# ORNL/HydraGNN

Measured on NVIDIA H100. Metric: atoms_per_sec_training_step, higher is better.
Workload: dtype tf32

## Files before the change

### hydragnn_b200/ops.py

```python
import torch
from torch.autograd.function import once_differentiable

from . import _lib

ACT_CODES = {None: 0, "none": 0, "relu": 1, "silu": 2, "tanh": 3, "sigmoid": 4, "lrelu": 5, "elu": 6, "selu": 7}
POOL_CODES = {"add": 0, "sum": 0, "mean": 1, "max": 2}


def _stream():
    return torch.cuda.current_stream().cuda_stream


def _p(t):
    return None if t is None else t.data_ptr()


def _chk(t, dtype=torch.float32):
    if t is None:
        return None
    if not t.is_cuda:
        raise RuntimeError("hydragnn_b200 ops need CUDA tensors (no CPU fallback on the hot path)")
    if t.dtype != dtype:
        raise RuntimeError("expected %s, got %s" % (dtype, t.dtype))
    return t if t.is_contiguous() else t.contiguous()
# ... 578 lines not shown
                                                leaves=ctx.leaves2)
            gx, gw1, gb1 = linear_bwd_dispatch(dz1, x2, w1, ctx.needs_input_grad[0], ctx.needs_input_grad[1],
                                               has_b1 and ctx.needs_input_grad[2], leaves=ctx.leaves1)
        return (gx.reshape(shp) if gx is not None else None), gw1, gb1, None, None, gw2, gb2, None, None


class Mlp2ScalarFn(torch.autograd.Function):

    @staticmethod
    def forward(ctx, x, w1, b1, act1, p1, w2, b2):
        n, out = x.shape[0], w2.shape[0]
        pad = x.new_zeros(4 - out)
        pk = torch.cat([w1.reshape(1), b1.reshape(1), w2.reshape(out), pad, b2.reshape(out), pad]).contiguous()
        x1 = _chk(x.reshape(n).contiguous())
        y = torch.empty(n, out, dtype=x.dtype, device=x.device)
        _lib.call("hgb_mlp2_scalar_fwd", _p(x1), _p(pk), n, out, ACT_CODES[act1], float(p1), _p(y), _stream())
        ctx.save_for_backward(x1, pk)
        ctx.cfg = (ACT_CODES[act1], float(p1), out)
        return y

    @staticmethod
    @once_differentiable
    def backward(ctx, gy):
        x1, pk = ctx.saved_tensors
        code, p1, out = ctx.cfg
        n = x1.shape[0]
        gx = torch.empty_like(x1) if ctx.needs_input_grad[0] else None
        gp = torch.empty(10, dtype=x1.dtype, device=x1.device)
        ws = _ws(_lib.query("hgb_mlp2_scalar_workspace_bytes"), x1.device)
        _lib.call("hgb_mlp2_scalar_bwd", _p(_chk(gy.contiguous())), _p(x1), _p(pk), n, out, code, p1, _p(gx), _p(gp), _p(ws), _stream())
        return (gx.reshape(n, 1) if gx is not None else None), gp[0:1].reshape(1, 1), gp[1:2], None, None, gp[2:2 + out].reshape(out, 1), gp[6:6 + out]


def mlp2(x, w1, b1, act1, p1, w2, b2, act2=None, p2=0.0):
    if (act2 is None and b1 is not None and b2 is not None and x.dim() == 2 and x.shape[1] == 1
            and w1.shape == (1, 1) and w2.shape[1] == 1 and w2.shape[0] <= 4):
        return Mlp2ScalarFn.apply(x, w1, b1, act1, p1, w2, b2)
    return Mlp2Fn.apply(x, w1, b1, act1, p1, w2, b2, act2, p2)


class EdgeGeomFn(torch.autograd.Function):

    @staticmethod
    def forward(ctx, pos, shifts, plan, eps):
        pos = _chk(pos)
        e = plan.num_edges
        vec = torch.empty(e, 3, dtype=pos.dtype, device=pos.device)
        ln = torch.empty(e, 1, dtype=pos.dtype, device=pos.device)
        unit = torch.empty(e, 3, dtype=pos.dtype, device=pos.device)
        _lib.call("hgb_edge_geom_fwd", _p(pos), _p(plan.row), _p(plan.col), _p(_chk(shifts)), e, float(eps), _p(vec), _p(ln),
                  _p(unit), _stream())
        ctx.save_for_backward(vec, ln)
        ctx.plan, ctx.eps = plan, float(eps)
        return vec, ln, unit

    @staticmethod
    @once_differentiable
    def backward(ctx, g_vec, g_len, g_unit):
        vec, ln = ctx.saved_tensors
        plan = ctx.plan
        gv = torch.empty_like(vec)
        _lib.call("hgb_edge_geom_bwd", _p(vec), _p(ln), ctx.eps, _p(_chk(g_vec)), _p(_chk(g_len)), _p(_chk(g_unit)),
                  plan.num_edges, _p(gv), _stream())
        g_pos = g_shift = None
        if ctx.needs_input_grad[0]:
            g_pos = raw_segment_sum(gv, plan.by_col.rowptr, plan.by_col.perm, plan.num_nodes) - \
                raw_segment_sum(gv, plan.by_row.rowptr, plan.by_row.perm, plan.num_nodes)
        if ctx.needs_input_grad[1]:
            g_shift = gv
        return g_pos, g_shift, None, None
# ... 60 lines not shown
            key = epack.data_ptr()
            if key not in cache:
                cache.clear()
                cache[key] = painn_edge_records(epack, plan, "col")
            rec_col = cache[key]
        _lib.call("hgb_painn_message_bwd", _p(gs_out), _p(gv_out), _p(phi), _p(v), _p(src.rowptr), _p(src.perm), _p(plan.nbr("col")),
                  _p(epack), _p(rec_col), _p(wf), _p(bf), _p(efilt), n, f, r, _p(gphi), _p(gv), _p(gwf), _p(gbf), _p(g_epack), _p(g_ef),
                  _p(ws), nbytes, _stream())
        return gphi, gs_out, gv, g_epack, gwf, gbf, g_ef, None, None


def painn_edge_records(epack, plan, which):
    csr = plan.by_row if which == "row" else plan.by_col
    rec = torch.empty(plan.num_edges, 16, dtype=epack.dtype, device=epack.device)
    _lib.call("hgb_painn_edge_records", _p(epack.detach()), _p(csr.perm), _p(plan.nbr(which)), plan.num_edges, _p(rec), _stream())
    return rec


def raw_linear(x2, w, b, code=0, param=0.0, want_z=False):
    m, k = x2.shape
    n = w.shape[0]
    y = torch.empty(m, n, dtype=x2.dtype, device=x2.device)
    z = torch.empty_like(y) if want_z else None
    _lib.call("hgb_linear_fwd", _p(x2), _p(w), _p(b), m, n, k, x2.stride(0), w.stride(0), code, float(param), _p(y), _p(z), _stream())
    return y, z


def raw_act_bwd(dy, y, z, code, param=0.0):
    dz = torch.empty_like(dy)
    _lib.call("hgb_act_bwd", _p(dy), _p(y), _p(z), dy.numel(), code, float(param), _p(dz), _stream())
    return dz


class PainnUpdateFn(torch.autograd.Function):

    @staticmethod
    def forward(ctx, s, v, uw, ub, vw, vb, w1, b1, w2, b2, last):
        n, f = s.shape
        s, v = _chk(s), _chk(v)
        w1, b1, w2, b2 = [_chk(t) for t in (w1, b1, w2, b2)]
        v2 = v.reshape(3 * n, f)
        wuv, buv = torch.cat([uw, vw], dim=0).contiguous(), torch.cat([ub, vb], dim=0).contiguous()
        y_uv, _ = linear_fwd_dispatch(v2, wuv, buv)
        uv, vv, ld = y_uv, y_uv[:, f:], 2 * f
        mlp_in = torch.empty(n, 2 * f, dtype=s.dtype, device=s.device)
        _lib.call("hgb_painn_update_pre_fwd", _p(vv), ld, _p(s), n, f, _p(mlp_in), _stream())
        h, z1, deriv = linear_fwd_dispatch_ex(mlp_in, w1, b1, ACT_CODES["silu"], 0.0, want_z=True, z_deriv=True)
        a, _ = linear_fwd_dispatch(h, w2, b2)
        ctx.z1_code = ACT_DERIV if deriv else ACT_CODES["silu"]
        s_out = torch.empty_like(s)
        v_out = None if last else torch.empty_like(v)
        _lib.call("hgb_painn_update_post_fwd", _p(a), _p(uv), _p(vv), ld, _p(s), _p(v), n, f, int(last), _p(s_out), _p(v_out), _stream())
        ctx.save_for_backward(v2, y_uv, mlp_in, z1, h, a, wuv, w1, w2)
        ctx.last = bool(last)
        ctx.tc = _TC["enabled"]
        ctx.leaves = ([uw, ub, vw, vb], [w1, b1], [w2, b2])
        if last:
            return s_out, s_out.new_zeros(0)
        return s_out, v_out

    @staticmethod
    @once_differentiable
    def backward(ctx, gs_out, gv_out):
        v2, y_uv, mlp_in, z1, h, a, wuv, w1, w2 = ctx.saved_tensors
        last = ctx.last
        n, f = gs_out.shape
        ld = 2 * f
        uv, vv = y_uv, y_uv[:, f:]
        gs_out = _chk(gs_out)
        gv_out = None if last else _chk(gv_out.contiguous())
        ga = torch.empty_like(a)
        _lib.call("hgb_painn_update_post_bwd_a", _p(gs_out), _p(gv_out), _p(uv), _p(vv), ld, n, f, int(last), _p(ga), _stream())
        with tensor_cores(ctx.tc):
            gz1, gw2, gb2 = linear_bwd_dispatch(ga, h, w2, dx_gsrc=z1, dx_gact=ctx.z1_code, leaves=ctx.leaves[2])
            g_mlp_in, gw1, gb1 = linear_bwd_dispatch(gz1, mlp_in, w1, leaves=ctx.leaves[1])
        g_uv = torch.empty_like(y_uv)
        gs = torch.empty_like(gs_out)
        _lib.call("hgb_painn_update_bwd", _p(gs_out), _p(gv_out), _p(g_mlp_in), _p(a), _p(uv), _p(vv), ld, _p(mlp_in), n, f,
                  int(last), _p(g_uv), _p(g_uv[:, f:]), _p(gs), None, _stream())
        with tensor_cores(ctx.tc):
            gv, gwuv, gbuv = linear_bwd_dispatch(g_uv, v2, wuv, dx_addend=None if last else gv_out.reshape(3 * n, f), leaves=ctx.leaves[0])
        return gs, gv.reshape(n, 3, f), gwuv[:f], gbuv[:f], gwuv[f:], gbuv[f:], gw1, gb1, gw2, gb2, None


def painn_update_tc_ok(s, v):
    n, f = s.shape
    return (_TC["enabled"] and f == 64 and tuple(v.shape) == (n, 3, f) and s.is_cuda and v.is_cuda
            and s.dtype == torch.float32 and v.dtype == torch.float32 and s.is_contiguous() and v.is_contiguous()
            and s.data_ptr() % 16 == 0 and v.data_ptr() % 16 == 0 and bool(_lib.query("hgb_tc_linear_supported", n, f, 2 * f)))


def _aligned(t):
    t = _chk(t)
    return t if t.data_ptr() % 16 == 0 else t.clone()


class PainnUpdateTcFn(torch.autograd.Function):

    @staticmethod
    def forward(ctx, s, v, uw, ub, vw, vb, w1, b1, w2, b2, last):
        n, f = s.shape
        w1, b1, w2, b2 = [_chk(t) for t in (w1, b1, w2, b2)]
        wuv, buv = torch.cat([uw, vw], dim=0).contiguous(), torch.cat([ub, vb], dim=0).contiguous()
        mlp_in = torch.empty(n, 2 * f, dtype=s.dtype, device=s.device)
        inner = torch.empty_like(s) if last else None
        _lib.call("hgb_painn_update_tc_fwd", _p(v), _p(s), _p(wuv), _p(buv), n, _p(mlp_in), _p(inner), _stream())
        h, z1, deriv = linear_fwd_dispatch_ex(mlp_in, w1, b1, ACT_CODES["silu"], 0.0, want_z=True, z_deriv=True)
        a, _ = linear_fwd_dispatch(h, w2, b2)
        ctx.z1_code = ACT_DERIV if deriv else ACT_CODES["silu"]
        s_out = torch.empty_like(s)
        v_out = None if last else torch.empty_like(v)
        _lib.call("hgb_painn_update_tc_post", _p(v), _p(s), _p(a), _p(inner), _p(wuv), _p(buv), n, int(last), _p(s_out), _p(v_out),
                  _stream())
        ctx.save_for_backward(v, mlp_in, z1, h, a, wuv, buv, w1, w2, inner)
        ctx.last = bool(last)
        ctx.leaves = ([uw, ub, vw, vb], [w1, b1], [w2, b2])
        if last:
            return s_out, s_out.new_zeros(0)
        return s_out, v_out

    @staticmethod
    @once_differentiable
    def backward(ctx, gs_out, gv_out):
        v, mlp_in, z1, h, a, wuv, buv, w1, w2, inner = ctx.saved_tensors
        last = ctx.last
        n, f = mlp_in.shape[0], v.shape[2]
        gs_out = _aligned(gs_out)
        gv_out = None if last else _aligned(gv_out)
        ga = torch.empty_like(a)
        _lib.call("hgb_painn_update_tc_bwd_a", _p(v), _p(gs_out), _p(gv_out), _p(inner), _p(wuv), _p(buv), n, int(last), _p(ga), _stream())
        with tensor_cores(True):
            gz1, gw2, gb2 = linear_bwd_dispatch(ga, h, w2, dx_gsrc=z1, dx_gact=ctx.z1_code, leaves=ctx.leaves[2])
            g_mlp_in, gw1, gb1 = linear_bwd_dispatch(gz1, mlp_in, w1, leaves=ctx.leaves[1])
        g_uv = torch.empty(3 * n, 2 * f, dtype=v.dtype, device=v.device)
        gs, gv = torch.empty_like(gs_out), torch.empty_like(v)
        _lib.call("hgb_painn_update_tc_bwd", _p(v), _p(gs_out), _p(gv_out), _p(g_mlp_in), _p(a), _p(mlp_in), _p(wuv), _p(buv), n, int(last),
                  _p(g_uv), _p(gs), _p(gv), _stream())
        with tensor_cores(True):
            _, gwuv, gbuv = linear_bwd_dispatch(g_uv, v.reshape(3 * n, f), wuv, need_x=False, leaves=ctx.leaves[0])
        return gs, gv, gwuv[:f], gbuv[:f], gwuv[f:], gbuv[f:], gw1, gb1, gw2, gb2, None


class PainnUpdateScalarFn(torch.autograd.Function):

    @staticmethod
    def forward(ctx, s, v, uw, ub, vw, vb, w1, b1, w2, b2, last):
        n = s.shape[0]
        na = 2 if last else 3
        pad = s.new_zeros(3 - na)
        pk = torch.cat([uw.reshape(1), ub.reshape(1), vw.reshape(1), vb.reshape(1), w1.reshape(2), b1.reshape(1), w2.reshape(na), pad,
                        b2.reshape(na), pad, s.new_zeros(3)]).contiguous()
        s2, v2 = _chk(s.reshape(n).contiguous()), _chk(v.reshape(n, 3).contiguous())
        s_out = torch.empty_like(s2)
        v_out = None if last else torch.empty_like(v2)
        _lib.call("hgb_painn_update_scalar_fwd", _p(s2), _p(v2), _p(pk), n, int(last), _p(s_out), _p(v_out), _stream())
        ctx.save_for_backward(s2, v2, pk)
        ctx.last = bool(last)
        if last:
            return s_out.reshape(n, 1), s_out.new_zeros(0)
        return s_out.reshape(n, 1), v_out.reshape(n, 3, 1)

    @staticmethod
    @once_differentiable
    def backward(ctx, gs_out, gv_out):
        s2, v2, pk = ctx.saved_tensors
        n, last = s2.shape[0], ctx.last
# ... 679 lines not shown
```

### include/hgb.h

```cpp
#ifndef HGB_H
#define HGB_H

#include <stdint.h>

#ifdef __cplusplus
extern "C" {
#endif

typedef void* hgb_stream_t;

#define HGB_OK 0
#define HGB_EINVAL (-1)
#define HGB_ECUDA (-2)
#define HGB_ECAPACITY (-3)

#define HGB_ACT_DERIV 100
#define HGB_ACT_NONE 0
#define HGB_ACT_RELU 1
#define HGB_ACT_SILU 2
#define HGB_ACT_TANH 3
#define HGB_ACT_SIGMOID 4
#define HGB_ACT_LRELU 5
#define HGB_ACT_ELU 6
#define HGB_ACT_SELU 7
// ... 58 lines not shown
int hgb_segment_argminmax(const float* m, const int32_t* rowptr, const int32_t* perm, int32_t n, int32_t c,
                          int64_t* argmin, int64_t* argmax, hgb_stream_t stream);
int hgb_pool_fwd(const float* x, const int32_t* graph_ptr, int32_t g, int32_t c, int32_t mode,
                 float* out, int32_t* argmax, hgb_stream_t stream);
int hgb_pool_bwd(const float* gout, const int32_t* graph_ptr, const int32_t* argmax, int32_t n,
                 int32_t g, int32_t c, int32_t mode, float* gx, hgb_stream_t stream);


int hgb_gemm(const float* a, const float* b, float* c, int32_t m, int32_t n, int32_t k,
             int32_t trans_a, int32_t trans_b, int64_t lda, int64_t ldb, int64_t ldc, int32_t beta_one,
             void* workspace, int64_t workspace_bytes, hgb_stream_t stream);
int64_t hgb_gemm_workspace_bytes(int32_t m, int32_t n, int32_t k, int32_t trans_a);
int hgb_linear_fwd(const float* x, const float* w, const float* b, int32_t m, int32_t n, int32_t k,
                   int64_t ldx, int64_t ldw, int32_t act, float act_param, float* y, float* z,
                   hgb_stream_t stream);
int hgb_linear_smallk_supported(int32_t n, int32_t k);
int hgb_linear_smallk_fwd(const float* x, int64_t ldx, const float* w, int64_t ldw, const float* b, int32_t m,
                          int32_t n, int32_t k, int32_t act, float act_param, float* y, float* z,
                          hgb_stream_t stream);
int hgb_linear_smallk_bwd(const float* dy, const float* y, const float* z, const float* x, int64_t ldx,
                          const float* w, int64_t ldw, int32_t m, int32_t n, int32_t k, int32_t act,
                          float act_param, float* dx, float* dw, int64_t lddw, float* db, void* workspace,
                          hgb_stream_t stream);
int64_t hgb_linear_smallk_bwd_workspace_bytes(int32_t m, int32_t n, int32_t k);

int hgb_tc_linear_supported(int32_t m, int32_t n_out, int32_t k_red);
int hgb_tc_linear(const float* a, int64_t lda, const float* w, int64_t ldw, int32_t trans_b, const float* bias,
                  int32_t m, int32_t n_out, int32_t k_red, int32_t act, float act_param, float* y, float* z,
                  const float* addend, const float* gsrc, int32_t gact, int32_t exact, hgb_stream_t stream);
int hgb_tc_wgrad(const float* dz, int64_t lddz, const float* x, int64_t ldx, int32_t m, int32_t n_out,
                 int32_t k_out, float* dw, int64_t lddw, float* db, int32_t accumulate, int32_t exact,
                 void* workspace, int64_t workspace_bytes, hgb_stream_t stream);
int64_t hgb_tc_wgrad_workspace_bytes(int32_t n_out, int32_t k_out);
int hgb_act_bwd(const float* dy, const float* y, const float* z, int64_t count, int32_t act,
                float act_param, float* dz, hgb_stream_t stream);
int hgb_act_deriv(const float* x, int64_t count, int32_t act, float act_param, int32_t order,
                  float* out, hgb_stream_t stream);
int hgb_colsum(const float* x, int32_t m, int32_t n, float* out, void* workspace, hgb_stream_t stream);
int64_t hgb_colsum_workspace_bytes(int32_t m, int32_t n);


int hgb_edge_geom_fwd(const float* pos, const int32_t* row, const int32_t* col, const float* shifts,
                      int64_t e, float eps, float* vec, float* len, float* unit, hgb_stream_t stream);
int hgb_edge_geom_bwd(const float* vec, const float* len, float eps, const float* g_vec_in,
                      const float* g_len, const float* g_unit, int64_t e, float* g_vec,
                      hgb_stream_t stream);
int hgb_painn_edge_embed_fwd(const float* unit, const float* len, int64_t e, int32_t r, float cutoff,
                             float* epack, hgb_stream_t stream);
int hgb_painn_edge_embed_bwd(const float* unit, const float* len, const float* g_epack, int64_t e, int32_t r,
                             float cutoff, float* g_unit, float* g_len, hgb_stream_t stream);


int hgb_painn_message_fwd(const float* phi, const float* s, const float* v, const int32_t* rowptr,
                          const int32_t* perm, const int32_t* nbr, const float* epack, const float* rec,
                          const float* wf, const float* bf, const float* efilt, int32_t n, int32_t f, int32_t r,
                          float* s_out, float* v_out, hgb_stream_t stream);
int hgb_painn_edge_records(const float* epack, const int32_t* perm, const int32_t* nbr, int64_t e, float* rec,
                           hgb_stream_t stream);
int hgb_painn_message_bwd(const float* gs_out, const float* gv_out, const float* phi, const float* v,
                          const int32_t* rowptr_src, const int32_t* perm_src, const int32_t* nbr_agg,
                          const float* epack, const float* rec, const float* wf, const float* bf, const float* efilt, int32_t n,
                          int32_t f, int32_t r, float* gphi, float* gv, float* gwf, float* gbf, float* g_epack,
                          float* g_efilt, void* workspace, int64_t workspace_bytes, hgb_stream_t stream);
int64_t hgb_painn_message_bwd_workspace_bytes(int32_t n, int32_t f, int32_t r);

int hgb_painn_update_pre_fwd(const float* vv, int64_t ld, const float* s, int32_t n, int32_t f, float* mlp_in,
// ... 152 lines not shown
```

### profiles/kbench.py

```python
import os, sys, json
sys.path.insert(0, os.path.dirname(os.path.dirname(os.path.abspath(__file__))))
import torch
import hydragnn_b200 as hb
from hydragnn_b200 import ops
from hydragnn_b200.stacks import Base
from hydragnn_b200.synthetic import ARCH, make_samples

dev = torch.device("cuda")
flush = torch.empty(256 * 1024 * 1024, dtype=torch.uint8, device=dev)


def timeit(fn, iters=10, warm=3):
    ts = []
    for it in range(iters + warm):
        flush.zero_()
        a, b = torch.cuda.Event(enable_timing=True), torch.cuda.Event(enable_timing=True)
        a.record(); fn(); b.record(); torch.cuda.synchronize()
        if it >= warm:
            ts.append(a.elapsed_time(b))
    return sum(ts) / len(ts)


def tc_linear_calls(n):
    silu, tanh, deriv = ops.ACT_CODES["silu"], ops.ACT_CODES["tanh"], ops.ACT_DERIV
# ... 21 lines not shown
        res["tc_linear %s m=%d (ms | GB/s)" % (name, m)] = (round(t, 4), round(nbytes / t / 1e6, 1))
    return res


def painn_update_calls(n, f=64):
    from hydragnn_b200.stacks import PainnUpdate
    units = {("fused", True): (19, 44), ("fused", False): (25, 56), ("unfused", True): (32, 58), ("unfused", False): (40, 72)}
    U = n * f * 4
    res = {}
    overlap = ops.WGRAD_OVERLAP
    ops.WGRAD_OVERLAP = False
    try:
        for last in (True, False):
            upd = PainnUpdate(f, last).to(dev)
            params = [upd.update_U.weight, upd.update_U.bias, upd.update_V.weight, upd.update_V.bias, upd.update_mlp[0].weight,
                      upd.update_mlp[0].bias, upd.update_mlp[2].weight, upd.update_mlp[2].bias]
            s = torch.randn(n, f, device=dev, requires_grad=True)
            v = torch.randn(n, 3, f, device=dev, requires_grad=True)
            for kind, fn in (("fused", ops.PainnUpdateTcFn), ("unfused", ops.PainnUpdateFn)):
                with ops.tensor_cores(True):
                    so, vo = fn.apply(s, v, *params, last)
                    outs = (so,) if last else (so, vo)
                    grads = tuple(torch.randn_like(o) for o in outs)
                    t_f = timeit(lambda: fn.apply(s, v, *params, last))
                    t_b = timeit(lambda: torch.autograd.grad(outs, [s, v] + params, grads, retain_graph=True))
                uf, ub = units[(kind, last)]
                res["painn_update %s last=%s fwd (ms | GB/s | U)" % (kind, last)] = (round(t_f, 4), round(uf * U / t_f / 1e6, 1), uf)
                res["painn_update %s last=%s bwd (ms | GB/s | U)" % (kind, last)] = (round(t_b, 4), round(ub * U / t_b / 1e6, 1), ub)
    finally:
        ops.WGRAD_OVERLAP = overlap
    return res


G = 16384
b = make_samples("qm9_painn", G).to(dev); b._num_graphs = G
if os.environ.get("KBENCH_ONLY") == "tc_linear":
    print(json.dumps(tc_linear_calls(b.pos.shape[0]), indent=1)); sys.exit(0)
if os.environ.get("KBENCH_ONLY") == "painn_update":
    print(json.dumps(painn_update_calls(b.pos.shape[0]), indent=1)); sys.exit(0)
b = hb.get_radius_graph(7.0, 5)(b)
plan = Base.plan_for(b)
n, e, f, r = plan.num_nodes, plan.num_edges, 64, 5
_, ln, unit = ops.EdgeGeomFn.apply(b.pos, None, plan, 1e-9)
epack = ops.PainnEdgeEmbedFn.apply(unit, ln, r, 7.0)
s, v, phi = torch.randn(n, f, device=dev), torch.randn(n, 3, f, device=dev), torch.randn(n, 3 * f, device=dev)
wf, bf = torch.randn(3 * f, r, device=dev), torch.randn(3 * f, device=dev)
out = {}
rec = ops.painn_edge_records(epack, plan, "row")
out["painn_message_fwd F=64 (ms)"] = timeit(lambda: ops.PainnMessageFn.apply(phi, s, v, epack, wf, bf, None, plan, rec))
out["painn_edge_records (ms)"] = timeit(lambda: ops.painn_edge_records(epack, plan, "row"))
sr, vr, pr = s.clone().requires_grad_(True), v.clone().requires_grad_(True), phi.clone().requires_grad_(True)
so, vo = ops.PainnMessageFn.apply(pr, sr, vr, epack, wf.requires_grad_(True), bf.requires_grad_(True), None, plan, rec)
gs, gv = torch.randn_like(so), torch.randn_like(vo)
out["painn_message_bwd F=64 (ms)"] = timeit(lambda: torch.autograd.grad((so, vo), (pr, sr, vr, wf, bf), (gs, gv), retain_graph=True))
so2, vo2 = ops.PainnMessageFn.apply(pr, sr, vr, epack, wf, bf, None, plan, None)
out["painn_message_bwd generic F=64 (ms)"] = timeit(lambda: torch.autograd.grad((so2, vo2), (pr, sr, vr, wf, bf), (gs, gv), retain_graph=True))
if os.environ.get("KBENCH_ONLY") == "painn":
    print(json.dumps(out, indent=1)); sys.exit(0)
alg_f = e * (6 * f * 4 + 8 + 48) + n * (8 * f * 4 + 4)
out["painn_message_fwd GB/s algorithmic"] = alg_f / out["painn_message_fwd F=64 (ms)"] / 1e6
for (m, k, nn_) in [(n, 64, 64), (n, 64, 192), (3 * n, 64, 64), (n, 128, 64), (n, 192, 64)]:
    x, w, bb = torch.randn(m, k, device=dev), torch.randn(nn_, k, device=dev), torch.randn(nn_, device=dev)
    t = timeit(lambda: ops.raw_tc_linear(x, w, False, bb, nn_, k))
    out["tc_linear m=%d k=%d n=%d (ms | GB/s)" % (m, k, nn_)] = (t, m * (k + nn_) * 4 / t / 1e6)
out.update(tc_linear_calls(n))
for (m, nn_, k) in [(n, 64, 64), (n, 192, 64), (3 * n, 64, 64)]:
    dz, x = torch.randn(m, nn_, device=dev), torch.randn(m, k, device=dev)
    t = timeit(lambda: ops.raw_tc_wgrad(dz, x))
# ... 3 lines not shown
```

Before: 41.42 million.

## Add fused two-layer MLP tensor-core kernels with warp-specialized TMA pipeline

Adds new Hopper wgmma/TMA kernels that compute a whole Linear-act-Linear MLP (hidden width 64) in one pass, keeping the hidden activation in shared memory. Forward no longer writes h/z1 to global memory, and backward recomputes h from x while fusing the dgrad of both layers, emitting h and dz1 for the weight gradients. The PaiNN update path now routes its MLP through these helpers. This targets memory traffic and launch count in the MLP stages, at the cost of recomputation in backward and extra shared-memory pressure.

```diff
diff --git a/hydragnn_b200/csrc/hgb_mlp_tc.cu b/hydragnn_b200/csrc/hgb_mlp_tc.cu
--- /dev/null
+++ b/hydragnn_b200/csrc/hgb_mlp_tc.cu
@@ -0,0 +1,478 @@
+#include "hgb_tc.cuh"
+
+namespace {
+
+constexpr int MH = 64;
+constexpr int MROWS = 64;
+constexpr uint32_t BOX = MROWS * 128;
+constexpr uint32_t HT = MROWS * MH * 4;
+constexpr int M2_THREADS = 384;
+constexpr int M2B_THREADS = 256;
+
+enum { A_NONE, A_RELU, A_SILU, A_TANH, A_OTHER };
+
+__device__ __forceinline__ float m2_act(float v, int kind, int act, float p, float& d) {
+  switch (kind) {
+    case A_SILU: {
+      const float s = __fdividef(1.f, 1.f + __expf(-v));
+      v *= s;
+      d = fmaf(v, 1.f - s, s);
+      return v;
+    }
+    case A_NONE: d = 1.f; return v;
+    case A_RELU: v = fmaxf(v, 0.f); break;
+    case A_TANH: v = tanhf(v); break;
+    default: v = hgb_act(v, act, p);
+  }
+  d = hgb_act_grad(v, v, act, p);
+  return v;
+}
+
+
+__device__ __forceinline__ void named_bar_arrive(int id, int threads) { asm volatile("bar.arrive %0, %1;" ::"r"(id), "r"(threads) : "memory"); }
+
+struct M2Params {
+  int m;
+  const float* w1;
+  const float* b1;
+  const float* w2;
+  const float* b2;
+  int act, kind;
+  float act_param;
+  float* y;
+  const float* x;
+  const float* dy;
+  float* gx;
+  float* h_out;
+  float* dz1_out;
+  int stages;
+};
+
+constexpr size_t fwd_smem(int k, int o, int sr) {
+  return 1024 + (size_t)k * 256 + (size_t)o * 256 + 2 * (size_t)HT + 2 * (size_t)sr * k * 256 + 4 * (size_t)sr * 8 + (size_t)(MH + o) * 4;
+}
+constexpr int fwd_stages(int k, int o) {
+  int s = 0;
+  for (int c = 1; c <= 4; ++c)
+    if (fwd_smem(k, o, c) <= SMEM_MAX) s = c;
+  return s;
+}
+constexpr size_t bwd_smem(int k, int o, int s) {
+  return 1024 + 2 * (size_t)k * 256 + (size_t)o * 256 + 2 * (size_t)HT + (size_t)s * (k + o) * 256 + (size_t)s * 8 + MH * 4;
+}
+constexpr int bwd_stages(int k, int o) {
+  int s = 0;
+  for (int c = 1; c <= 4; ++c)
+    if (bwd_smem(k, o, c) <= SMEM_MAX) s = c;
+  return s;
+}
+
+__device__ __forceinline__ void stage_w(uint8_t* dst, uint8_t* dst_t, const float* w, int rows, int cols, int t0, int nt) {
+  constexpr int SU = 8;
+  const int total = rows * cols;
+  for (int base = t0; base < total; base += nt * SU) {
+    float v[SU];
+#pragma unroll
+    for (int u = 0; u < SU; ++u) {
+      const int i = base + u * nt;
+      v[u] = i < total ? __ldg(w + i) : 0.f;
+    }
+#pragma unroll
+    for (int u = 0; u < SU; ++u) {
+      const int i = base + u * nt;
+      if (i < total) {
+        const int r = i / cols, c = i - r * cols;
+        if (dst) *reinterpret_cast<float*>(dst + kmajor_sw128_off(r, c, rows)) = v[u];
+        if (dst_t) *reinterpret_cast<float*>(dst_t + kmajor_sw128_off(c, r, cols)) = v[u];
+      }
+    }
+  }
+}
+
+__device__ __forceinline__ void prefetch_l2(const float* p, uint32_t bytes) {
+  asm volatile("cp.async.bulk.prefetch.L2.global [%0], %1;" ::"l"(p), "r"(bytes) : "memory");
+}
+
+}
+
+template <int KB, int OC>
+__global__ void __launch_bounds__(M2_THREADS, 1) mlp2_fwd_kernel(const __grid_constant__ CUtensorMap tmap_x, const M2Params p) {
+  constexpr int K = KB * 32, O = OC * 32;
+  constexpr uint32_t XS = KB * BOX;
+  extern __shared__ uint8_t smem_raw[];
+  uint8_t* smem = reinterpret_cast<uint8_t*>((reinterpret_cast<uintptr_t>(smem_raw) + 1023) & ~(uintptr_t)1023);
+  uint8_t* sB1 = smem;
+  uint8_t* sB2 = sB1 + K * 256;
+  uint8_t* sH = sB2 + O * 256;
+  uint8_t* sX = sH + 2 * HT;
+  const int SR = p.stages;
+  uint64_t* full = reinterpret_cast<uint64_t*>(sX + (size_t)2 * SR * XS);
+  uint64_t* empty = full + 2 * SR;
+  float* sb1 = reinterpret_cast<float*>(empty + 2 * SR);
+  float* sb2 = sb1 + MH;
+
+  const int warp = threadIdx.x >> 5, lane = threadIdx.x & 31;
+  const int ntiles = (p.m + MROWS - 1) / MROWS;
+  for (int i = threadIdx.x; i < MH; i += blockDim.x) sb1[i] = p.b1 ? __ldg(p.b1 + i) : 0.f;
+  for (int i = threadIdx.x; i < O; i += blockDim.x) sb2[i] = p.b2 ? __ldg(p.b2 + i) : 0.f;
+  if (threadIdx.x == 0) {
+    for (int s = 0; s < 2 * SR; ++s) { mbar_init(full + s, 1); mbar_init(empty + s, 4); }
+    fence_barrier_init();
+  }
+  __syncthreads();
+
+  if (warp < 4) {
+    regs_dec<PRODUCER_REGS>();
+    if (warp == 0 && lane == 0) {
+      uint32_t li = 0;
+      for (int t = blockIdx.x; t < ntiles; t += gridDim.x, ++li) {
+        const uint32_t n = li >> 1;
+        const int s = (li & 1) * SR + n % SR;
+        mbar_wait(empty + s, ((n / SR) & 1) ^ 1);
+        mbar_expect_tx(full + s, XS);
+        for (int kb = 0; kb < KB; ++kb) tma_load_2d(sX + (size_t)s * XS + kb * BOX, &tmap_x, full + s, kb * 32, t * MROWS);
+      }
+    }
+    return;
+  }
+  regs_inc<CONSUMER_REGS>();
+  stage_w(sB1, nullptr, p.w1, MH, K, threadIdx.x - 128, 256);
+  stage_w(sB2, nullptr, p.w2, O, MH, threadIdx.x - 128, 256);
+  fence_proxy_async();
+  named_bar_sync(1, 256);
+
+  const int cw = (warp - 4) >> 2, wq = warp & 3;
+  const int rsub = wq * 16 + (lane >> 2), c2 = 2 * (lane & 3);
+  uint8_t* sHo = sH + cw * HT;
+  const uint32_t sX_addr = smem_u32(sX), sB1_addr = smem_u32(sB1), sB2_addr = smem_u32(sB2), sH_addr = smem_u32(sHo);
+  float acc1[32], acc2[OC * 16];
+  int li = cw;
+  for (int t = blockIdx.x + cw * gridDim.x; t < ntiles; t += 2 * gridDim.x, li += 2) {
+    const uint32_t n = (uint32_t)li >> 1;
+    const int s = cw * SR + n % SR;
+    mbar_wait(full + s, (n / SR) & 1);
+#pragma unroll
+    for (int j = 0; j < 32; ++j) acc1[j] = 0.f;
+    fence_regs<32>(acc1);
+    wgmma_fence();
+#pragma unroll
+    for (int kb = 0; kb < KB; ++kb)
+#pragma unroll
+      for (int k4 = 0; k4 < 4; ++k4)
+        wgmma_tf32<2>(acc1, make_desc(sX_addr + s * XS + kb * BOX + k4 * 32), make_desc(sB1_addr + kb * MH * 128 + k4 * 32));
+    wgmma_commit();
+    wgmma_wait<0>();
+    fence_regs<32>(acc1);
+    __syncwarp();
+    if (lane == 0) mbar_arrive(empty + s);
+    named_bar_sync(2 + cw, 128);
+#pragma unroll
+    for (int j = 0; j < 32; j += 2) {
+      const int r = rsub + 8 * ((j >> 1) & 1), col = 8 * (j >> 2) + c2;
+      float d0, d1;
+      const float h0 = m2_act(acc1[j] + sb1[col], p.kind, p.act, p.act_param, d0);
+      const float h1 = m2_act(acc1[j + 1] + sb1[col + 1], p.kind, p.act, p.act_param, d1);
+      *reinterpret_cast<float2*>(sHo + kmajor_sw128_off(r, col, MROWS)) = make_float2(h0, h1);
+    }
+    fence_proxy_async();
+    named_bar_sync(2 + cw, 128);
+#pragma unroll
+    for (int j = 0; j < OC * 16; ++j) acc2[j] = 0.f;
+    fence_regs<OC * 16>(acc2);
+    wgmma_fence();
+#pragma unroll
+    for (int jb = 0; jb < 2; ++jb)
+#pragma unroll
+      for (int k4 = 0; k4 < 4; ++k4)
+        wgmma_tf32<OC>(acc2, make_desc(sH_addr + jb * BOX + k4 * 32), make_desc(sB2_addr + jb * O * 128 + k4 * 32));
+    wgmma_commit();
+    wgmma_wait<0>();
+    fence_regs<OC * 16>(acc2);
+    const int row0 = t * MROWS;
+#pragma unroll
+    for (int h = 0; h < 2; ++h) {
+      const int row = row0 + rsub + 8 * h;
+      if (row < p.m) {
+        float* yr = p.y + (int64_t)row * O + c2;
+#pragma unroll
+        for (int i = 0; i < OC * 4; ++i) {
+          const int col = 8 * i + c2;
+          *reinterpret_cast<float2*>(yr + 8 * i) = make_float2(acc2[4 * i + 2 * h] + sb2[col], acc2[4 * i + 2 * h + 1] + sb2[col + 1]);
+        }
+      }
+    }
+  }
+}
+
+template <int KB, int OC>
+__global__ void __launch_bounds__(M2B_THREADS, 1) mlp2_bwd_kernel(const __grid_constant__ CUtensorMap tmap_x, const __grid_constant__ CUtensorMap tmap_dy,
+                                                                 const M2Params p) {
+  constexpr int K = KB * 32, O = OC * 32;
+  constexpr uint32_t TS = (KB + OC) * BOX;
+  extern __shared__ uint8_t smem_raw[];
+  uint8_t* smem = reinterpret_cast<uint8_t*>((reinterpret_cast<uintptr_t>(smem_raw) + 1023) & ~(uintptr_t)1023);
+  uint8_t* sB1 = smem;
+  uint8_t* sB1t = sB1 + K * 256;
+  uint8_t* sB2t = sB1t + K * 256;
+  uint8_t* sH = sB2t + O * 256;
+  uint8_t* sD = sH + HT;
+  uint8_t* sT = sD + HT;
+  const int S = p.stages;
+  uint64_t* full = reinterpret_cast<uint64_t*>(sT + (size_t)S * TS);
+  float* sb1 = reinterpret_cast<float*>(full + S);
+
+  const int warp = threadIdx.x >> 5, lane = threadIdx.x & 31;
+  const int ntiles = (p.m + MROWS - 1) / MROWS;
+  for (int i = threadIdx.x; i < MH; i += blockDim.x) sb1[i] = p.b1 ? __ldg(p.b1 + i) : 0.f;
+  if (threadIdx.x == 0) {
+    for (int s = 0; s < S; ++s) mbar_init(full + s, 1);
+    fence_barrier_init();
+  }
+  __syncthreads();
+  const bool issuer = threadIdx.x == 128;
+  auto load = [&](int tt, int s) {
+    mbar_expect_tx(full + s, TS);
+    uint8_t* st = sT + (size_t)s * TS;
+    for (int kb = 0; kb < KB; ++kb) tma_load_2d(st + kb * BOX, &tmap_x, full + s, kb * 32, tt * MROWS);
+    for (int ob = 0; ob < OC; ++ob) tma_load_2d(st + (KB + ob) * BOX, &tmap_dy, full + s, ob * 32, tt * MROWS);
+  };
+  auto prefetch = [&](int tt) {
+    if (tt < ntiles) {
+      const int rows = min(MROWS, p.m - tt * MROWS);
+      prefetch_l2(p.x + (int64_t)tt * MROWS * K, (uint32_t)rows * K * 4);
+      prefetch_l2(p.dy + (int64_t)tt * MROWS * O, (uint32_t)rows * O * 4);
+    }
+  };
+  if (issuer) {
+    for (int s = 0; s < S; ++s)
+      if (blockIdx.x + s * (int)gridDim.x < ntiles) load(blockIdx.x + s * gridDim.x, s);
+    prefetch(blockIdx.x + S * gridDim.x);
+  }
+  stage_w(sB1, sB1t, p.w1, MH, K, threadIdx.x, M2B_THREADS);
+  stage_w(nullptr, sB2t, p.w2, O, MH, threadIdx.x, M2B_THREADS);
+  fence_proxy_async();
+  __syncthreads();
+  const int wg = warp >> 2, wq = warp & 3;
+
+  if (wg == 0) {
+    const int rsub = wq * 16 + (lane >> 2), c2 = 2 * (lane & 3);
+    const uint32_t sT_addr = smem_u32(sT), sB1_addr = smem_u32(sB1), sB1t_addr = smem_u32(sB1t), sB2t_addr = smem_u32(sB2t),
+                   sD_addr = smem_u32(sD);
+    float acc1[32], accd[32], dv[32], accg[KB * 16];
+    uint32_t c = 0;
+    for (int t = blockIdx.x; t < ntiles; t += gridDim.x, ++c) {
+      const int s = c % S;
+      const uint32_t st = sT_addr + s * TS;
+      mbar_wait(full + s, (c / S) & 1);
+#pragma unroll
+      for (int j = 0; j < 32; ++j) acc1[j] = accd[j] = 0.f;
+      fence_regs<32>(acc1);
+      fence_regs<32>(accd);
+      wgmma_fence();
+#pragma unroll
+      for (int kb = 0; kb < KB; ++kb)
+#pragma unroll
+        for (int k4 = 0; k4 < 4; ++k4)
+          wgmma_tf32<2>(acc1, make_desc(st + kb * BOX + k4 * 32), make_desc(sB1_addr + kb * MH * 128 + k4 * 32));
+      wgmma_commit();
+#pragma unroll
+      for (int ob = 0; ob < OC; ++ob)
+#pragma unroll
+        for (int k4 = 0; k4 < 4; ++k4)
+          wgmma_tf32<2>(accd, make_desc(st + (KB + ob) * BOX + k4 * 32), make_desc(sB2t_addr + ob * MH * 128 + k4 * 32));
+      wgmma_commit();
+      wgmma_wait<1>();
+      fence_regs<32>(acc1);
+#pragma unroll
+      for (int j = 0; j < 32; ++j) acc1[j] = m2_act(acc1[j] + sb1[8 * (j >> 2) + c2 + (j & 1)], p.kind, p.act, p.act_param, dv[j]);
+      if (c > 0) named_bar_sync(4, 256);
+#pragma unroll
+      for (int j = 0; j < 32; j += 2) {
+        const int r = rsub + 8 * ((j >> 1) & 1), col = 8 * (j >> 2) + c2;
+        *reinterpret_cast<float2*>(sH + kmajor_sw128_off(r, col, MROWS)) = make_float2(acc1[j], acc1[j + 1]);
+      }
+      named_bar_arrive(2, 256);
+      wgmma_wait<0>();
+      fence_regs<32>(accd);
+#pragma unroll
+      for (int j = 0; j < 32; j += 2) {
+        const int r = rsub + 8 * ((j >> 1) & 1), col = 8 * (j >> 2) + c2;
+        *reinterpret_cast<float2*>(sD + kmajor_sw128_off(r, col, MROWS)) = make_float2((accd[j] + 0.f) * dv[j], (accd[j + 1] + 0.f) * dv[j + 1]);
+      }
+      fence_proxy_async();
+      named_bar_sync(1, 128);
+      named_bar_arrive(3, 256);
+#pragma unroll
+      for (int j = 0; j < KB * 16; ++j) accg[j] = 0.f;
+      fence_regs<KB * 16>(accg);
+      wgmma_fence();
+#pragma unroll
+      for (int jb = 0; jb < 2; ++jb)
+#pragma unroll
+        for (int k4 = 0; k4 < 4; ++k4)
+          wgmma_tf32<KB>(accg, make_desc(sD_addr + jb * BOX + k4 * 32), make_desc(sB1t_addr + jb * K * 128 + k4 * 32));
+      wgmma_commit();
+      wgmma_wait<0>();
+      fence_regs<KB * 16>(accg);
+      if (p.gx) {
+#pragma unroll
+        for (int h = 0; h < 2; ++h) {
+          const int row = t * MROWS + rsub + 8 * h;
+          if (row < p.m) {
+            float* gr = p.gx + (int64_t)row * K + c2;
+#pragma unroll
+            for (int i = 0; i < KB * 4; ++i)
+              *reinterpret_cast<float2*>(gr + 8 * i) = make_float2(accg[4 * i + 2 * h] + 0.f, accg[4 * i + 2 * h + 1] + 0.f);
+          }
+        }
+      }
+    }
+    return;
+  }
+
+  uint32_t c = 0;
+  const int tw = threadIdx.x - 128;
+  for (int t = blockIdx.x; t < ntiles; t += gridDim.x, ++c) {
+    const int s = c % S;
+    const int row0 = t * MROWS;
+    named_bar_sync(2, 256);
+#pragma unroll
+    for (int i = 0; i < MROWS * MH / 4 / 128; ++i) {
+      const int idx = i * 128 + tw, r = idx >> 4, col = (idx & 15) * 4;
+      if (row0 + r < p.m)
+        *reinterpret_cast<float4*>(p.h_out + (int64_t)(row0 + r) * MH + col) =
+            *reinterpret_cast<const float4*>(sH + kmajor_sw128_off(r, col, MROWS));
+    }
+    named_bar_sync(3, 256);
+    if (issuer && t + S * (int)gridDim.x < ntiles) {
+      load(t + S * gridDim.x, s);
+      prefetch(t + (S + 1) * gridDim.x);
+    }
+#pragma unroll
+    for (int i = 0; i < MROWS * MH / 4 / 128; ++i) {
+      const int idx = i * 128 + tw, r = idx >> 4, col = (idx & 15) * 4;
+      if (row0 + r < p.m)
+        *reinterpret_cast<float4*>(p.dz1_out + (int64_t)(row0 + r) * MH + col) =
+            *reinterpret_cast<const float4*>(sD + kmajor_sw128_off(r, col, MROWS));
+    }
+    if (t + (int)gridDim.x < ntiles) named_bar_arrive(4, 256);
+  }
+}
+
+namespace {
+
+bool m2_shape(int k, int h, int o) { return h == MH && k >= 32 && k <= 128 && k % 32 == 0 && o >= 32 && o <= 256 && o % 32 == 0; }
+bool m2_fits(int k, int o) { return fwd_stages(k, o) >= 1 && bwd_stages(k, o) >= 1; }
+bool al16(const void* q) { return ((uintptr_t)q & 15) == 0; }
+
+int m2_kind(int act) {
+  return act == HGB_ACT_NONE ? A_NONE : act == HGB_ACT_RELU ? A_RELU : act == HGB_ACT_SILU ? A_SILU : act == HGB_ACT_TANH ? A_TANH : A_OTHER;
+}
+
+template <int KB, int OC>
+void launch_fwd_t(const CUtensorMap& tx, const M2Params& p, cudaStream_t st) {
+  constexpr int SR = fwd_stages(KB * 32, OC * 32);
+  constexpr size_t smem = fwd_smem(KB * 32, OC * 32, SR);
+  static bool attr = false;
+  if (!attr) {
+    cudaFuncSetAttribute(mlp2_fwd_kernel<KB, OC>, cudaFuncAttributeMaxDynamicSharedMemorySize, (int)smem);
+    attr = true;
+  }
+  M2Params q = p;
+  q.stages = SR;
+  const int ntiles = (p.m + MROWS - 1) / MROWS;
+  const int grid = (ntiles + 1) / 2 < HGB_NUM_SMS ? (ntiles + 1) / 2 : HGB_NUM_SMS;
+  mlp2_fwd_kernel<KB, OC><<<grid, M2_THREADS, smem, st>>>(tx, q);
+}
+
+template <int KB, int OC>
+int launch_bwd_t(const CUtensorMap& tx, const CUtensorMap& tdy, const M2Params& p, cudaStream_t st) {
+  constexpr int S = bwd_stages(KB * 32, OC * 32);
+  if constexpr (S >= 1) {
+    constexpr size_t smem = bwd_smem(KB * 32, OC * 32, S);
+    static bool attr = false;
+    if (!attr) {
+      cudaFuncSetAttribute(mlp2_bwd_kernel<KB, OC>, cudaFuncAttributeMaxDynamicSharedMemorySize, (int)smem);
+      attr = true;
+    }
+    M2Params q = p;
+    q.stages = S;
+    const int ntiles = (p.m + MROWS - 1) / MROWS;
+    const int grid = ntiles < HGB_NUM_SMS ? ntiles : HGB_NUM_SMS;
+    mlp2_bwd_kernel<KB, OC><<<grid, M2B_THREADS, smem, st>>>(tx, tdy, q);
+    return grid;
+  } else {
+    return 0;
+  }
+}
+
+template <template <int, int> class F, int KB, typename... A>
+int m2_dispatch_o(int oc, A&&... a) {
+  switch (oc) {
+    case 1: return F<KB, 1>::run(a...);
+    case 2: return F<KB, 2>::run(a...);
+    case 3: return F<KB, 3>::run(a...);
+    case 4: return F<KB, 4>::run(a...);
+    case 5: return F<KB, 5>::run(a...);
+    case 6: return F<KB, 6>::run(a...);
+    case 7: return F<KB, 7>::run(a...);
+    default: return F<KB, 8>::run(a...);
+  }
+}
+template <template <int, int> class F, typename... A>
+int m2_dispatch(int kb, int oc, A&&... a) {
+  switch (kb) {
+    case 1: return m2_dispatch_o<F, 1>(oc, a...);
+    case 2: return m2_dispatch_o<F, 2>(oc, a...);
+    case 3: return m2_dispatch_o<F, 3>(oc, a...);
+    default: return m2_dispatch_o<F, 4>(oc, a...);
+  }
+}
+template <int KB, int OC>
+struct FwdLaunch {
+  static int run(const CUtensorMap& tx, const M2Params& p, cudaStream_t st) { launch_fwd_t<KB, OC>(tx, p, st); return 0; }
+};
+template <int KB, int OC>
+struct BwdLaunch {
+  static int run(const CUtensorMap& tx, const CUtensorMap& tdy, const M2Params& p, cudaStream_t st) { return launch_bwd_t<KB, OC>(tx, tdy, p, st); }
+};
+
+}
+
+extern "C" int hgb_mlp2_tc_supported(int32_t k, int32_t h, int32_t o) { return (m2_shape(k, h, o) && m2_fits(k, o)) ? 1 : 0; }
+
+extern "C" int hgb_mlp2_tc_fwd(const float* x, const float* w1, const float* b1, const float* w2, const float* b2, int32_t m, int32_t k,
+                               int32_t h, int32_t o, int32_t act, float act_param, float* y, hgb_stream_t stream) {
+  HGB_REQUIRE(m >= 0 && x && w1 && w2 && y && hgb_mlp2_tc_supported(k, h, o), "mlp2_tc_fwd: unsupported arguments m=%d k=%d h=%d o=%d", m, k, h,
+              o);
+  HGB_REQUIRE(al16(x) && al16(y), "mlp2_tc_fwd: x and y must be 16-byte aligned");
+  if (m == 0) return HGB_OK;
+  CUtensorMap tx;
+  int rc = make_tmap(&tx, x, m, k, k, MROWS, CU_TENSOR_MAP_SWIZZLE_128B);
+  if (rc) return rc;
+  M2Params p = {};
+  p.m = m; p.w1 = w1; p.b1 = b1; p.w2 = w2; p.b2 = b2; p.act = act; p.kind = m2_kind(act); p.act_param = act_param; p.y = y;
+  m2_dispatch<FwdLaunch>(k / 32, o / 32, tx, p, (cudaStream_t)stream);
+  HGB_LAUNCH_CHECK("mlp2_tc_fwd");
+  return HGB_OK;
+}
+
+extern "C" int hgb_mlp2_tc_bwd(const float* dy, const float* x, const float* w1, const float* b1, const float* w2, int32_t m, int32_t k,
+                               int32_t h, int32_t o, int32_t act, float act_param, float* gx, float* h_out, float* dz1, hgb_stream_t stream) {
+  HGB_REQUIRE(m >= 0 && dy && x && w1 && w2 && h_out && dz1 && hgb_mlp2_tc_supported(k, h, o), "mlp2_tc_bwd: unsupported arguments m=%d k=%d h=%d o=%d",
+              m, k, h, o);
+  HGB_REQUIRE(al16(dy) && al16(x) && al16(gx) && al16(h_out) && al16(dz1), "mlp2_tc_bwd: dy, x, gx, h and dz1 must be 16-byte aligned");
+  if (m == 0) return HGB_OK;
+  CUtensorMap tx, tdy;
+  int rc = make_tmap(&tx, x, m, k, k, MROWS, CU_TENSOR_MAP_SWIZZLE_128B);
+  if (rc) return rc;
+  rc = make_tmap(&tdy, dy, m, o, o, MROWS, CU_TENSOR_MAP_SWIZZLE_128B);
+  if (rc) return rc;
+  M2Params p = {};
+  p.m = m; p.w1 = w1; p.b1 = b1; p.w2 = w2; p.act = act; p.kind = m2_kind(act); p.act_param = act_param; p.gx = gx; p.x = x; p.dy = dy;
+  p.h_out = h_out;
+  p.dz1_out = dz1;
+  m2_dispatch<BwdLaunch>(k / 32, o / 32, tx, tdy, p, (cudaStream_t)stream);
+  HGB_LAUNCH_CHECK("mlp2_tc_bwd");
+  return HGB_OK;
+}
diff --git a/hydragnn_b200/ops.py b/hydragnn_b200/ops.py
--- a/hydragnn_b200/ops.py
+++ b/hydragnn_b200/ops.py
@@ -634,10 +634,74 @@
         return (gx.reshape(n, 1) if gx is not None else None), gp[0:1].reshape(1, 1), gp[1:2], None, None, gp[2:2 + out].reshape(out, 1), gp[6:6 + out]
 
 
+def _dense_f32(t, align=1):
+    return t is None or (t.is_cuda and t.dtype == torch.float32 and t.is_contiguous() and t.data_ptr() % align == 0)
+
+
+def mlp2_tc_ok(x, w1, b1, w2, b2, act2=None):
+    if not _TC["enabled"] or act2 is not None or x.dim() < 1 or w1.dim() != 2 or w2.dim() != 2:
+        return False
+    k, h, o = x.shape[-1], w1.shape[0], w2.shape[0]
+    m = x.numel() // k if k else 0
+    return (w1.shape[1] == k and w2.shape[1] == h and _dense_f32(x, 16) and all(_dense_f32(t) for t in (w1, b1, w2, b2))
+            and bool(_lib.query("hgb_mlp2_tc_supported", k, h, o)) and bool(_lib.query("hgb_tc_linear_supported", m, h, k)))
+
+
+def raw_mlp2_tc_fwd(x2, w1, b1, code, param, w2, b2):
+    m, k = x2.shape
+    y = torch.empty(m, w2.shape[0], dtype=x2.dtype, device=x2.device)
+    _lib.call("hgb_mlp2_tc_fwd", _p(x2), _p(w1), _p(b1), _p(w2), _p(b2), m, k, w1.shape[0], w2.shape[0], code, float(param), _p(y), _stream())
+    return y
+
+
+def raw_mlp2_tc_bwd(dy, x2, w1, b1, w2, code, param, need_x=True):
+    m, k = x2.shape
+    gx = torch.empty_like(x2) if need_x else None
+    h = torch.empty(m, w1.shape[0], dtype=x2.dtype, device=x2.device)
+    dz1 = torch.empty_like(h)
+    _lib.call("hgb_mlp2_tc_bwd", _p(dy), _p(x2), _p(w1), _p(b1), _p(w2), m, k, w1.shape[0], w2.shape[0], code, float(param), _p(gx), _p(h),
+              _p(dz1), _stream())
+    return gx, h, dz1
+
+
+def mlp2_tc_bwd(dy, x2, w1, b1, w2, code, param, need_x, need, leaves):
+    gx, h, dz1 = raw_mlp2_tc_bwd(dy, x2, w1, b1, w2, code, param, need_x)
+    with tensor_cores(True):
+        _, gw2, gb2 = linear_bwd_dispatch(dy, h, w2, need_x=False, need_w=need[2], need_b=need[3], leaves=leaves[1])
+        _, gw1, gb1 = linear_bwd_dispatch(dz1, x2, w1, need_x=False, need_w=need[0], need_b=need[1], leaves=leaves[0])
+    return gx, gw1, gb1, gw2, gb2
+
+
+class Mlp2TcFn(torch.autograd.Function):
+
+    @staticmethod
+    def forward(ctx, x, w1, b1, act1, p1, w2, b2):
+        shp = x.shape
+        x2 = x.reshape(-1, shp[-1])
+        code = ACT_CODES[act1]
+        y = raw_mlp2_tc_fwd(x2, w1, b1, code, p1, w2, b2)
+        ctx.save_for_backward(x2, w1, b1, w2)
+        ctx.cfg = (code, float(p1), shp, b1 is not None, b2 is not None)
+        ctx.leaves = ([w1] + ([b1] if b1 is not None else []), [w2] + ([b2] if b2 is not None else []))
+        return y.reshape(shp[:-1] + (w2.shape[0],))
+
+    @staticmethod
+    @once_differentiable
+    def backward(ctx, gy):
+        x2, w1, b1, w2 = ctx.saved_tensors
+        code, p1, shp, has_b1, has_b2 = ctx.cfg
+        gy2 = _aligned(gy.reshape(x2.shape[0], w2.shape[0]))
+        need = (ctx.needs_input_grad[1], has_b1 and ctx.needs_input_grad[2], ctx.needs_input_grad[5], has_b2 and ctx.needs_input_grad[6])
+        gx, gw1, gb1, gw2, gb2 = mlp2_tc_bwd(gy2, x2, w1, b1, w2, code, p1, ctx.needs_input_grad[0], need, ctx.leaves)
+        return (gx.reshape(shp) if gx is not None else None), gw1, gb1, None, None, gw2, gb2
+
+
 def mlp2(x, w1, b1, act1, p1, w2, b2, act2=None, p2=0.0):
     if (act2 is None and b1 is not None and b2 is not None and x.dim() == 2 and x.shape[1] == 1
             and w1.shape == (1, 1) and w2.shape[1] == 1 and w2.shape[0] <= 4):
         return Mlp2ScalarFn.apply(x, w1, b1, act1, p1, w2, b2)
+    if mlp2_tc_ok(x, w1, b1, w2, b2, act2):
+        return Mlp2TcFn.apply(x, w1, b1, act1, p1, w2, b2)
     return Mlp2Fn.apply(x, w1, b1, act1, p1, w2, b2, act2, p2)
 
 
@@ -764,6 +828,22 @@
     return dz
 
 
+def _update_mlp_fwd(mlp_in, w1, b1, w2, b2):
+    if mlp2_tc_ok(mlp_in, w1, b1, w2, b2):
+        return raw_mlp2_tc_fwd(mlp_in, w1, b1, ACT_CODES["silu"], 0.0, w2, b2), None, None, None
+    h, z1, deriv = linear_fwd_dispatch_ex(mlp_in, w1, b1, ACT_CODES["silu"], 0.0, want_z=True, z_deriv=True)
+    a, _ = linear_fwd_dispatch(h, w2, b2)
+    return a, z1, h, (ACT_DERIV if deriv else ACT_CODES["silu"])
+
+
+def _update_mlp_bwd(ga, mlp_in, z1, h, w1, b1, w2, z1_code, leaves):
+    if h is None:
+        return mlp2_tc_bwd(ga, mlp_in, w1, b1, w2, ACT_CODES["silu"], 0.0, True, (True,) * 4, (leaves[1], leaves[2]))
+    gz1, gw2, gb2 = linear_bwd_dispatch(ga, h, w2, dx_gsrc=z1, dx_gact=z1_code, leaves=leaves[2])
+    g_mlp_in, gw1, gb1 = linear_bwd_dispatch(gz1, mlp_in, w1, leaves=leaves[1])
+    return g_mlp_in, gw1, gb1, gw2, gb2
+
+
 class PainnUpdateFn(torch.autograd.Function):
 
     @staticmethod
@@ -777,13 +857,11 @@
         uv, vv, ld = y_uv, y_uv[:, f:], 2 * f
         mlp_in = torch.empty(n, 2 * f, dtype=s.dtype, device=s.device)
         _lib.call("hgb_painn_update_pre_fwd", _p(vv), ld, _p(s), n, f, _p(mlp_in), _stream())
-        h, z1, deriv = linear_fwd_dispatch_ex(mlp_in, w1, b1, ACT_CODES["silu"], 0.0, want_z=True, z_deriv=True)
-        a, _ = linear_fwd_dispatch(h, w2, b2)
-        ctx.z1_code = ACT_DERIV if deriv else ACT_CODES["silu"]
+        a, z1, h, ctx.z1_code = _update_mlp_fwd(mlp_in, w1, b1, w2, b2)
         s_out = torch.empty_like(s)
         v_out = None if last else torch.empty_like(v)
         _lib.call("hgb_painn_update_post_fwd", _p(a), _p(uv), _p(vv), ld, _p(s), _p(v), n, f, int(last), _p(s_out), _p(v_out), _stream())
-        ctx.save_for_backward(v2, y_uv, mlp_in, z1, h, a, wuv, w1, w2)
+        ctx.save_for_backward(v2, y_uv, mlp_in, z1, h, a, wuv, w1, b1, w2)
         ctx.last = bool(last)
         ctx.tc = _TC["enabled"]
         ctx.leaves = ([uw, ub, vw, vb], [w1, b1], [w2, b2])
@@ -794,7 +872,7 @@
     @staticmethod
     @once_differentiable
     def backward(ctx, gs_out, gv_out):
-        v2, y_uv, mlp_in, z1, h, a, wuv, w1, w2 = ctx.saved_tensors
+        v2, y_uv, mlp_in, z1, h, a, wuv, w1, b1, w2 = ctx.saved_tensors
         last = ctx.last
         n, f = gs_out.shape
         ld = 2 * f
@@ -804,8 +882,7 @@
         ga = torch.empty_like(a)
         _lib.call("hgb_painn_update_post_bwd_a", _p(gs_out), _p(gv_out), _p(uv), _p(vv), ld, n, f, int(last), _p(ga), _stream())
         with tensor_cores(ctx.tc):
-            gz1, gw2, gb2 = linear_bwd_dispatch(ga, h, w2, dx_gsrc=z1, dx_gact=ctx.z1_code, leaves=ctx.leaves[2])
-            g_mlp_in, gw1, gb1 = linear_bwd_dispatch(gz1, mlp_in, w1, leaves=ctx.leaves[1])
+            g_mlp_in, gw1, gb1, gw2, gb2 = _update_mlp_bwd(ga, mlp_in, z1, h, w1, b1, w2, ctx.z1_code, ctx.leaves)
         g_uv = torch.empty_like(y_uv)
         gs = torch.empty_like(gs_out)
         _lib.call("hgb_painn_update_bwd", _p(gs_out), _p(gv_out), _p(g_mlp_in), _p(a), _p(uv), _p(vv), ld, _p(mlp_in), n, f,
@@ -837,14 +914,12 @@
         mlp_in = torch.empty(n, 2 * f, dtype=s.dtype, device=s.device)
         inner = torch.empty_like(s) if last else None
         _lib.call("hgb_painn_update_tc_fwd", _p(v), _p(s), _p(wuv), _p(buv), n, _p(mlp_in), _p(inner), _stream())
-        h, z1, deriv = linear_fwd_dispatch_ex(mlp_in, w1, b1, ACT_CODES["silu"], 0.0, want_z=True, z_deriv=True)
-        a, _ = linear_fwd_dispatch(h, w2, b2)
-        ctx.z1_code = ACT_DERIV if deriv else ACT_CODES["silu"]
+        a, z1, h, ctx.z1_code = _update_mlp_fwd(mlp_in, w1, b1, w2, b2)
         s_out = torch.empty_like(s)
         v_out = None if last else torch.empty_like(v)
         _lib.call("hgb_painn_update_tc_post", _p(v), _p(s), _p(a), _p(inner), _p(wuv), _p(buv), n, int(last), _p(s_out), _p(v_out),
                   _stream())
-        ctx.save_for_backward(v, mlp_in, z1, h, a, wuv, buv, w1, w2, inner)
+        ctx.save_for_backward(v, mlp_in, z1, h, a, wuv, buv, w1, b1, w2, inner)
         ctx.last = bool(last)
         ctx.leaves = ([uw, ub, vw, vb], [w1, b1], [w2, b2])
         if last:
@@ -854,7 +929,7 @@
     @staticmethod
     @once_differentiable
     def backward(ctx, gs_out, gv_out):
-        v, mlp_in, z1, h, a, wuv, buv, w1, w2, inner = ctx.saved_tensors
+        v, mlp_in, z1, h, a, wuv, buv, w1, b1, w2, inner = ctx.saved_tensors
         last = ctx.last
         n, f = mlp_in.shape[0], v.shape[2]
         gs_out = _aligned(gs_out)
@@ -862,8 +937,7 @@
         ga = torch.empty_like(a)
         _lib.call("hgb_painn_update_tc_bwd_a", _p(v), _p(gs_out), _p(gv_out), _p(inner), _p(wuv), _p(buv), n, int(last), _p(ga), _stream())
         with tensor_cores(True):
-            gz1, gw2, gb2 = linear_bwd_dispatch(ga, h, w2, dx_gsrc=z1, dx_gact=ctx.z1_code, leaves=ctx.leaves[2])
-            g_mlp_in, gw1, gb1 = linear_bwd_dispatch(gz1, mlp_in, w1, leaves=ctx.leaves[1])
+            g_mlp_in, gw1, gb1, gw2, gb2 = _update_mlp_bwd(ga, mlp_in, z1, h, w1, b1, w2, ctx.z1_code, ctx.leaves)
         g_uv = torch.empty(3 * n, 2 * f, dtype=v.dtype, device=v.device)
         gs, gv = torch.empty_like(gs_out), torch.empty_like(v)
         _lib.call("hgb_painn_update_tc_bwd", _p(v), _p(gs_out), _p(gv_out), _p(g_mlp_in), _p(a), _p(mlp_in), _p(wuv), _p(buv), n, int(last),
diff --git a/include/hgb.h b/include/hgb.h
--- a/include/hgb.h
+++ b/include/hgb.h
@@ -114,6 +114,12 @@
                  int32_t k_out, float* dw, int64_t lddw, float* db, int32_t accumulate, int32_t exact,
                  void* workspace, int64_t workspace_bytes, hgb_stream_t stream);
 int64_t hgb_tc_wgrad_workspace_bytes(int32_t n_out, int32_t k_out);
+int hgb_mlp2_tc_supported(int32_t k, int32_t h, int32_t o);
+int hgb_mlp2_tc_fwd(const float* x, const float* w1, const float* b1, const float* w2, const float* b2, int32_t m,
+                    int32_t k, int32_t h, int32_t o, int32_t act, float act_param, float* y, hgb_stream_t stream);
+int hgb_mlp2_tc_bwd(const float* dy, const float* x, const float* w1, const float* b1, const float* w2, int32_t m,
+                    int32_t k, int32_t h, int32_t o, int32_t act, float act_param, float* gx, float* h_out, float* dz1,
+                    hgb_stream_t stream);
 int hgb_act_bwd(const float* dy, const float* y, const float* z, int64_t count, int32_t act,
                 float act_param, float* dz, hgb_stream_t stream);
 int hgb_act_deriv(const float* x, int64_t count, int32_t act, float act_param, int32_t order,
diff --git a/profiles/kbench.py b/profiles/kbench.py
--- a/profiles/kbench.py
+++ b/profiles/kbench.py
@@ -77,8 +77,43 @@
     return res
 
 
+def mlp2_calls(n):
+    U = n * 64 * 4
+    res = {}
+    overlap = ops.WGRAD_OVERLAP
+    ops.WGRAD_OVERLAP = False
+    try:
+        for name, k, o, act in (("message_mlp", 64, 192, "silu"), ("node_embed_out", 64, 64, "tanh"),
+                                ("update_mlp last", 128, 128, "silu"), ("update_mlp", 128, 192, "silu")):
+            kx, oy = k / 64, o / 64
+            z = 1 if act == "silu" else 0
+            units = {"fused": (kx + oy, (2 * kx + oy + 2) + (oy + 1) + (1 + kx)),
+                     "Mlp2Fn": (kx + 2 + z + oy, (oy + 2) + (oy + 1) + (1 + kx) + (1 + kx))}
+            x = torch.randn(n, k, device=dev, requires_grad=True)
+            w1, b1 = (torch.randn(64, k, device=dev) / k ** 0.5).requires_grad_(True), torch.randn(64, device=dev, requires_grad=True)
+            w2, b2 = (torch.randn(o, 64, device=dev) / 8).requires_grad_(True), torch.randn(o, device=dev, requires_grad=True)
+            for kind in ("fused", "Mlp2Fn"):
+                def fwd():
+                    if kind == "fused":
+                        return ops.Mlp2TcFn.apply(x, w1, b1, act, 0.0, w2, b2)
+                    return ops.Mlp2Fn.apply(x, w1, b1, act, 0.0, w2, b2, None, 0.0)
+                with ops.tensor_cores(True):
+                    y = fwd()
+                    gy = torch.randn_like(y)
+                    t_f = timeit(fwd)
+                    t_b = timeit(lambda: torch.autograd.grad(y, [x, w1, b1, w2, b2], gy, retain_graph=True))
+                uf, ub = units[kind]
+                res["mlp2 %s %d->64->%d %s %s fwd (ms | GB/s | U)" % (name, k, o, act, kind)] = (round(t_f, 4), round(uf * U / t_f / 1e6, 1), uf)
+                res["mlp2 %s %d->64->%d %s %s bwd (ms | GB/s | U)" % (name, k, o, act, kind)] = (round(t_b, 4), round(ub * U / t_b / 1e6, 1), ub)
+    finally:
+        ops.WGRAD_OVERLAP = overlap
+    return res
+
+
 G = 16384
 b = make_samples("qm9_painn", G).to(dev); b._num_graphs = G
+if os.environ.get("KBENCH_ONLY") == "mlp2":
+    print(json.dumps(mlp2_calls(b.pos.shape[0]), indent=1)); sys.exit(0)
 if os.environ.get("KBENCH_ONLY") == "tc_linear":
     print(json.dumps(tc_linear_calls(b.pos.shape[0]), indent=1)); sys.exit(0)
 if os.environ.get("KBENCH_ONLY") == "painn_update":
```

After: 44.36 million, median of 6. 1.07x the previous value.
